# agussomacal/ROMHighContrast

Measured on AMD Instinct MI355X. Metric: snapshot_solves_per_sec, higher is better.
Workload: dtype f64

## Files before the change

romhighcontrast_amd/csrc/rom_fem_dev.h:

```cpp
#pragma once
#include "rom_fem_plan.h"
#include "rom_mma.h"

struct FemDev {
  int nrb, ncb, N, n1, n1p, nr, nc, nGp, nGa, T, nslots, kblk, npre, nrhs, nexp, ncross, xb0;
  long long dim;
  const double* pool;
  const int* alist;
  const int* aoff;
  int tile_stream;
  const int* pairs;
  int npairs;
  const double* pool_acc;
  const int* wmeta;
  int wp0[5];
  int s1_t0, s1_nterm, s1_ndr;
  const int* s1_items;
  const int* s1_citems;
  const GenTerm* terms;
  const double* Bt;
  const double* P;
  const double* vec;
  const RhsTerm* rhs;
  const PreEdge* pre;
// ... 33 lines not shown
  const int* colti;
  const BlockSide* sides;
  int n_lr;
  const int* lr_blocks;
  const int* gen_blocks;
  const int* vmap;
  const int* scat;
  int nscat;
  double* L;
  double* invL;
  double* y;
  int* status;
};


FemDev make_dev(const rom_fem* f);

constexpr int S1_COEF_BYTES = 4 * COEF_MAX * 8, S1_WAVE_BYTES = (40 * 64 + 64 * 4 + 64 + 64 + 3 * 64 * 4) * 8;
constexpr int S1_ITEM_PASSES = 4;
constexpr int S1_DENSE_BYTES = 64 * 64 * 8;
constexpr int S1_LDS_BYTES = S1_COEF_BYTES + 4 * S1_WAVE_BYTES + S1_DENSE_BYTES;

__global__ void k_repack_table(const double* __restrict__ G, int ld, int nseg, int n1, int orient, double* __restrict__ Gs);
__global__ void k_build_A0(double* A0, const double* Qp, const double* rho, int n1, int n1p, int N);
__global__ void k_rhs(FemDev f, const double* __restrict__ a);
__global__ void k_coef(FemDev f, const double* __restrict__ a);
__global__ void k_expand(FemDev f, const double* __restrict__ a, int Mc, double* __restrict__ U, long long row0);
__global__ void k_back_pre(FemDev f, const double* __restrict__ a, int Mc);
template <int NS>
__global__ void k_diag_update(FemDev f, const double* __restrict__ a, int slot, int Mc);
__global__ void k_diag_factor(FemDev f, int slot, int j);
__global__ void k_solve1(FemDev f, const double* __restrict__ a, int Mc);
template <int NS>
__global__ void k_factor_panel(FemDev f, const double* __restrict__ a, int j, int Mc);
__global__ void k_backsolve(FemDev f);
__global__ void k_edge_transform(FemDev f, int Mc);
__global__ void k_extend(FemDev f, const double* __restrict__ a, int Mc, double* __restrict__ U, long long row0, const int* __restrict__ blocks, int pw_log2);
struct X128Args {
  int blocks[X128_BLOCKS];
  BlockSide sides[X128_BLOCKS];
};

template <bool FLAT>
__global__ void k_extend128(FemDev f, X128Args xa, const double* __restrict__ a, int Mc, double* __restrict__ U, long long row0, int with_expand, int sys_fast);
__device__ inline void load4_any(const double* __restrict__ p, double v[4]) {
  if (p) {
// ... 64 lines not shown
```

romhighcontrast_amd/csrc/rom_fem_kernels.hip:

```cpp
#include "rom_fem_dev.h"

__global__ void k_build_A0(double* A0, const double* Qp, const double* rho, int n1, int n1p, int N) {
  size_t idx = blockIdx.x * size_t(blockDim.x) + threadIdx.x;
  size_t total = size_t(n1) * n1 * n1p;
  if (idx >= total) return;
  int m = int(idx % n1p);
  size_t ij = idx / n1p;
  int j = int(ij % n1) + 1, i = int(ij / n1) + 1;
  A0[idx] = (m < n1) ? Qp[size_t(j - 1) * n1p + m] * rho[size_t(m) * (N + 1) + i] : 0.0;
}

__global__ void k_repack_table(const double* __restrict__ G, int ld, int nseg, int n1, int orient, double* __restrict__ Gs) {
  const long long idx = blockIdx.x * (long long)blockDim.x + threadIdx.x;
  const long long hrows = (long long)n1 * n1;
  if (idx >= (long long)nseg * hrows * 8) return;
  const int kk = int(idx & 7);
  const long long rp = (idx >> 3) % hrows, seg = (idx >> 3) / hrows;
  const long long row = orient ? (rp % n1) * n1 + rp / n1 : rp;
  const int k = int(seg) * 8 + kk;
  Gs[idx] = k < ld ? G[row * ld + k] : 0.0;
}


__device__ inline double readlane_f64(double v, int lane) {
  int lo = __builtin_amdgcn_readlane(__double2loint(v), lane);
  int hi = __builtin_amdgcn_readlane(__double2hiint(v), lane);
  return __hiloint2double(hi, lo);
}

__device__ inline double term_coef(const GenTerm& g, const double* __restrict__ am) {
  switch (g.kind) {
    case 0: return -am[g.b[0]];
    case 1: return am[g.b[0]] + am[g.b[1]];
    case 2: return -(am[g.b[0]] + am[g.b[1]]) / 2;
    case 3: return ((am[g.b[0]] + am[g.b[1]]) + am[g.b[2]]) + am[g.b[3]];
    case 4: return -(am[g.b[0]] * am[g.b[1]] / (am[g.b[2]] + am[g.b[3]]));
    case 5: return -(am[g.b[0]] / 2);
    default: return -((am[g.b[2]] + am[g.b[3]]) / 4);
  }
}

struct STile {
  double v[16];
// ... 1416 lines not shown
    const int cidx = acc_col(wp, jb);
    const int wi = i0 + (cidx >> pw_log2) - 1, wj = j0 + (cidx & (pw - 1)) - 1;
    w_own[jb] = (wi < n1 && wj < n1) ? f.W[wi * n1 + wj] : 0.0;
  }
#pragma unroll
  for (int i = 0; i < 2; ++i)
#pragma unroll
    for (int g = 0; g < 4; ++g) {
      const int m = blockIdx.y * 64 + acc_row(wp, i, g);
      const double sc = scs[acc_row(wp, i, g)];
      const double x0 = acc.c[i][0][g] + sc * w_own[0], x1 = acc.c[i][1][g] + sc * w_own[1];
      const double got = lane_swap1(odd ? x0 : x1);
      if (m >= Mc) continue;
      double* dst = U + (row0 + m) * f.dim + gidx;
      const double lo = odd ? got : x0, hi = odd ? x1 : got;
      if (v1) *reinterpret_cast<double2_u*>(dst) = double2_u{lo, hi};
      else if (v0) dst[0] = lo;
    }
}



constexpr int X128_SLOT = 4 * 128 * 64;

template <bool FLAT>
__global__ __launch_bounds__(512, 2) void k_extend128(FemDev f, X128Args xa, const double* __restrict__ a, int Mc,
                                                      double* __restrict__ U, long long row0, int with_expand,
                                                      int sys_fast) {
  __shared__ __align__(16) char lds_bytes[2 * X128_SLOT];
  __shared__ double scs[128];
  double* const lds = reinterpret_cast<double*>(lds_bytes);
  const int n1 = f.n1, N = f.N;
  const int nct = (n1 + 127) / 128;
  const int nvert = n1 * n1;
  const int ntile = FLAT ? (nvert + 127) / 128 : n1 * nct;
  int bx, by, ngy;
  if (sys_fast > 0) {
    bx = int(blockIdx.x) / sys_fast; by = int(blockIdx.x) % sys_fast; ngy = sys_fast;
  } else if (sys_fast < 0) {
    ngy = -sys_fast;
    const int unit = int(blockIdx.x) / (8 * ngy), r = int(blockIdx.x) % (8 * ngy);
    bx = unit * 8 + (r & 7); by = r >> 3;
  } else {
    bx = int(blockIdx.x); by = int(blockIdx.y); ngy = int(gridDim.y);
  }
  if (bx >= ntile + with_expand) return;
// ... 16 lines not shown
  const BlockSide sd = xa.sides[bz];
  const int iv = bx / nct + 1;
  const int jv0 = 128 * (bx % nct) + 1;
  const int vt0 = 128 * bx;
  const int lane = threadIdx.x & 63, w = __builtin_amdgcn_readfirstlane(threadIdx.x >> 6), wr = w >> 2, wc = w & 3;
  constexpr int NJ = 2;
  const int fr = lane & 15, kq = lane >> 4;
  double my_sc = 0.0;
  if (threadIdx.x < 128) {
    const int m = by * 128 + threadIdx.x;
    if (m < Mc) my_sc = f.y[size_t(m) * f.nGp + f.sblk0 + b];
  }
  double w_own[NJ];
#pragma unroll
  for (int j = 0; j < NJ; ++j) {
    if (FLAT) {
      const int v = vt0 + wc * (16 * NJ) + j * 16 + fr;
      w_own[j] = v < nvert ? f.W[v] : 0.0;
    } else {
      const int jj = jv0 + wc * (16 * NJ) + j * 16 + fr;
      w_own[j] = jj <= n1 ? f.W[(iv - 1) * n1 + (jj - 1)] : 0.0;
    }
  }
  const int cnt0 = sd.s[0].mode == 2 ? min(2 * sd.s[0].nch, (sd.s[0].r + 1 + 7) / 8) : 0;
  const int cnt1 = sd.s[1].mode == 2 ? min(2 * sd.s[1].nch, (sd.s[1].r + 1 + 7) / 8) : 0;
  const int cnt2 = sd.s[2].mode == 2 ? min(2 * sd.s[2].nch, (sd.s[2].r + 1 + 7) / 8) : 0;
  const int cnt3 = sd.s[3].mode == 2 ? min(2 * sd.s[3].nch, (sd.s[3].r + 1 + 7) / 8) : 0;
  const int nseg = cnt0 + cnt1 + cnt2 + cnt3;
  const int tot = (nseg + 1) / 2;
  const unsigned fx = unsigned((kq >> 1) ^ (fr >> 2));
  const unsigned fa0 = unsigned(fr * 64) + (fx << 4) + unsigned(kq & 1) * 8u;
  const unsigned fa1 = unsigned(fr * 64) + ((fx ^ 2u) << 4) + unsigned(kq & 1) * 8u;
#define X_FRAGS(SLOT_, KKI_, AF_, BF_)                                                                             \
  do {                                                                                                             \
    const char* pf_ = lds_bytes + (SLOT_) * X128_SLOT + (((KKI_)&1) ? fa1 : fa0);                                  \
    const char* pa_ = pf_ + ((KKI_) >> 1) * 8192 + wr * 4096;                                                      \
    const char* pb_ = pf_ + 16384 + ((KKI_) >> 1) * 8192 + wc * (1024 * NJ);                                       \
    _Pragma("unroll") for (int i_ = 0; i_ < 4; ++i_) AF_[i_] = *reinterpret_cast<const double*>(pa_ + i_ * 1024);  \
    _Pragma("unroll") for (int i_ = 0; i_ < NJ; ++i_) BF_[i_] = *reinterpret_cast<const double*>(pb_ + i_ * 1024); \
  } while (0)
  const unsigned lds0 = unsigned(size_t((__attribute__((address_space(3))) char*)lds_bytes));
  const unsigned du16 = unsigned(((lane & 3) ^ ((lane >> 4) & 3)) * 16);
  const unsigned ybytes_row = unsigned(f.nGp) * 8u;
  const int m0 = by * 128;
  unsigned voA[2];
  int vi[2], vj[2];
#pragma unroll
  for (int g = 0; g < 2; ++g) {
    const int rl = 32 * (w & 3) + 16 * g + (lane >> 2);
    voA[g] = unsigned(max(0, min(rl, Mc - 1 - m0))) * ybytes_row + du16;
// ... 7 lines not shown
    }
  }
  const char* const ybase = reinterpret_cast<const char*>(f.y) + size_t(min(m0, Mc - 1)) * ybytes_row;
  const char* const gsbase = reinterpret_cast<const char*>(f.Gs);
  const size_t seg_stride = size_t(n1) * n1 * 64;
  const char* const zbase = reinterpret_cast<const char*>(f.W + size_t(n1) * n1);
  const unsigned voZ = unsigned(lane) * 16u;
  int c_side = -1, c_left = 0, c_segs = nseg;
  const char* pA = zbase;
  const char* pB = zbase;
  unsigned voB[2] = {0, 0};
#define X_NEXT_SIDE()                                                                                              \
  do {                                                                                                             \
    do {                                                                                                           \
      ++c_side;                                                                                                    \
      c_left = c_side == 0 ? cnt0 : c_side == 1 ? cnt1 : c_side == 2 ? cnt2 : cnt3;                                \
    } while (c_left == 0 && c_side < 3);                                                                           \
    const int off_ = c_side == 0 ? sd.s[0].off : c_side == 1 ? sd.s[1].off : c_side == 2 ? sd.s[2].off : sd.s[3].off; \
    const int gseg_ = c_side == 0 ? sd.s[0].gseg : c_side == 1 ? sd.s[1].gseg : c_side == 2 ? sd.s[2].gseg : sd.s[3].gseg; \
     \
         \
    const int ci_ = c_side == 1 ? -n1 : n1, cj_ = c_side == 3 ? -1 : 1;                                             \
    const int k0_ = c_side == 1 ? n1 * n1 - 1 : c_side == 3 ? -n1 + n1 : -n1 - 1;                                   \
    pA = ybase + size_t(off_) * 8;                                                                                 \
    pB = gsbase + size_t(gseg_) * 8;                                                                               \
    voB[0] = unsigned(ci_ * vi[0] + cj_ * vj[0] + k0_) * 64u + du16;                                               \
    voB[1] = unsigned(ci_ * vi[1] + cj_ * vj[1] + k0_) * 64u + du16;                                               \
  } while (0)
#define X_DMA(LDS_, BASE_, VOFF_)                                                                                  \
  asm volatile("s_mov_b32 m0, %0\n\tglobal_load_lds_dwordx4 %1, %2" ::"s"(__builtin_amdgcn_readfirstlane(LDS_)),   \
               "v"(VOFF_), "s"(x128_uniform(BASE_))                                                                \
               : "memory", "m0")
#define X_ISSUE_HALF(SLOT_, H_, MINE_)                                                                             \
  do {                                                                                                             \
    const unsigned sb_ = lds0 + unsigned(SLOT_) * X128_SLOT + (H_) * 8192 + unsigned(w & 3) * 2048;                \
    if (c_segs > 0) {                                                                                              \
      if (MINE_) {                                                                                                 \
        X_DMA(sb_, pA, voA[0]);                                                                                    \
        X_DMA(sb_ + 1024, pA, voA[1]);                                                                             \
        X_DMA(sb_ + 16384, pB, voB[0]);                                                                            \
        X_DMA(sb_ + 16384 + 1024, pB, voB[1]);                                                                     \
      }                                                                                                            \
      pA += 64;                                                                                                    \
      pB += seg_stride;                                               \
      --c_segs;                                                                                                    \
      if (--c_left == 0 && c_segs > 0) X_NEXT_SIDE();                                                              \
    } else if (MINE_) {                                                 \
      X_DMA(sb_, zbase, voZ);                                                                                      \
// ... 148 lines not shown
```

romhighcontrast_amd/csrc/rom_fem_plan.h:

```cpp
#pragma once
#include <string>
#include <vector>

#include "romhc_internal.h"

constexpr int COEF_MAX = 64;
#ifndef PAIR_RING_
#define PAIR_RING_ 8
#endif
constexpr int PAIR_RING = PAIR_RING_;
constexpr int DENSE_GROUPS_MAX = 8;
constexpr int EXT_ZERO_PAGE = 256;
constexpr int X128_BLOCKS = 16;

__host__ __device__ inline int h0_row(int s, int i, int j, int N, int n1) {
  int ii, jj;
  switch (s) {
    case 0: ii = i; jj = j; break;
    case 1: ii = N - i; jj = j; break;
    case 2: ii = j; jj = i; break;
    default: ii = N - j; jj = i; break;
  }
  return (ii - 1) * n1 + (jj - 1);
}

struct FemSwitches {
  bool no_preelim, no_compress, no_lowrank_ext, no_ext_lr, verbose;
  long double compress_tol;
};

struct FemPlan {
  int nrb, ncb, N, n1, n1p, nr, nc, nG, nGp, nGa, nred, ncross, xb0, T, nslots, n_all_edges, npre_all;
  int64_t dim;
  int spos0, nsc, npairs = 0, wp0[5] = {}, ncoef, ncf, nctask, ndg, ndi, n_edges, lr_nch;
  bool fused1 = false;
  std::vector<double> pool, pool_acc, dmat, Ptab, Bt, Qp, rho, Wz, g_red, vecs, cm;
  std::vector<GenTerm> terms;
  std::vector<TileDesc> desc;
  std::vector<int> alist, aoff, pairs, wmeta, s1_items, s1_citems, dweight, ditem_group, ditem_k, kmax, item_group, item_k, item_cf;
  std::vector<int> ctask, xred, scb, kptr, kpair, colptr, colrow, colti, vmap, scat, lr_blocks, gen_blocks, epos;
  std::vector<DenseGroup> dgroups;
  std::vector<RhsTerm> rhs_terms;
  std::vector<PreEdge> pre_edges;
  std::vector<ExpEdge> exps;
  std::vector<CoefGroup> groups;
  std::vector<BlockSide> sides;
  struct GemmG { std::vector<double> Bh; long long off; int rp; };
  struct Repack { long long goff, gsoff; int ld, nseg, orient; };
  std::vector<GemmG> gemm_G;
  std::vector<Repack> repacks;
  long long gtotal = 0, gstotal = 0;
  std::vector<int> ranks, slot_of, diag_slot;
  double ext_flops = 0, flops_solve = 0, bytes_solve = 0;
};

int rom_fem_plan(int nrb, int ncb, int N, const FemSwitches& sw, FemPlan* out, std::string* error);
```

romhighcontrast_amd/csrc/rom_fem_plan.hip:

```cpp
#include "rom_fem_plan.h"

#include <algorithm>
#include <array>
#include <atomic>
#include <chrono>
#include <cmath>
#include <cstring>
#include <map>
#include <set>
#include <thread>
#include <tuple>

#include "rom_hostla.h"

namespace {

using hostla::ld;
using hostla::Mat;

struct Edge {
  int hv, p, q;
  int b0, b1;
};

struct Small {
  int rpos, cpos;
  Mat tab;
  int kind;
  std::array<int, 4> b;
};

struct Comp {
  int r = 0;
  Mat W;
  Mat Kt;
  Mat P;
  std::vector<ld> gt;
  std::vector<ld> p0;
  Mat KiW;
  std::vector<ld> wK;
};

template <class F>
void parallel_for(size_t n, F fn) {
  const unsigned nthr = std::max(1u, std::min<unsigned>(std::thread::hardware_concurrency(), unsigned(n)));
  std::atomic<size_t> next{0};
  auto work = [&]() {
    for (size_t i = next++; i < n; i = next++) fn(i);
  };
  std::vector<std::thread> pool;
  for (unsigned t = 1; t < nthr; ++t) pool.emplace_back(work);
  work();
  for (auto& th : pool) th.join();
}

struct UnitBlock {
  int N, n1;
  Mat Q, rho;
  std::vector<ld> lam, kappa;
  Mat Wl;
  Mat Kmat, Kinv;
  std::vector<ld> gE[2];
  std::vector<double> rho_d, Wd;
// ... 122 lines not shown
  }
  Mat Wb(n1, r);
  for (int i = 0; i < n1; ++i)
    for (int k = 0; k < r; ++k) Wb(i, k) = Wfull(i, k);
  cp.r = r;
  cp.W = Wb;
  Mat KiW = hostla::mul(ub.Kinv, Wb);
  Mat G = hostla::mul_tn(Wb, KiW);
  for (int i = 0; i < G.r; ++i)
    for (int j = 0; j < i; ++j) G(i, j) = G(j, i) = (G(i, j) + G(j, i)) / 2;
  if (!hostla::spd_inverse(G, cp.Kt)) return false;
  cp.P = hostla::mul(KiW, cp.Kt);
  std::vector<ld> v = hostla::matvec(ub.Kinv, ub.gE[hv]);
  std::vector<ld> wv = hostla::matvec(hostla::transpose(Wb), v);
  cp.gt = hostla::matvec(cp.Kt, wv);
  std::vector<ld> pw = hostla::matvec(cp.P, wv);
  cp.p0.resize(n1);
  for (int i = 0; i < n1; ++i) cp.p0[i] = v[i] - pw[i];
  cp.KiW = KiW;
  cp.wK = v;
  return true;
}

struct TermAcc {
  std::array<int, 5> key;
  std::vector<double> tab;
  int r_lo, r_hi, c_lo, c_hi;
};

void put_table(std::vector<double>& pool, size_t idx, int n1p, const Mat& A, bool transposed) {
  double* dst = pool.data() + idx * size_t(n1p) * n1p;
  for (int i = 0; i < A.r; ++i)
    for (int j = 0; j < A.c; ++j) {
      if (transposed) dst[size_t(j) * n1p + i] = double(A(i, j));
      else dst[size_t(i) * n1p + j] = double(A(i, j));
    }
}

int pad_bk(int r) { return (r + 1 + BK - 1) / BK * BK; }
int segs8(int r) { return (r + 1 + 7) / 8; }

int push_vec(std::vector<double>& vecs, const std::vector<ld>& v, int padded) {
  const int off = int(vecs.size());
  for (ld x : v) vecs.push_back(double(x));
  for (int i = int(v.size()); i < padded; ++i) vecs.push_back(0.0);
  return off;
// ... 118 lines not shown
    for (int e = 0; e < E; ++e) {
      if (done[e] || is_pre[e]) continue;
      if (best < 0 || g[e].size() < bd) { best = e; bd = g[e].size(); }
    }
    done[best] = 1;
    el.ord_of[best] = int(el.order.size());
    el.order.push_back(best);
    std::vector<int> nb(g[best].begin(), g[best].end());
    for (int x : nb) {
      g[x].erase(best);
      for (int y : nb)
        if (x != y) g[x].insert(y);
    }
  }
  return el;
}

struct Compression {
  std::vector<std::vector<int>> sigs;
  std::vector<int> comp_of;
  std::vector<Comp> comps;
  std::vector<int> kmax, rp;
  std::vector<char> use_lr;
  double kavg = 0;
};

void edge_types(const Topology& t, Compression& c) {
  std::map<std::vector<int>, int> sig_id;
  c.comp_of.assign(t.E, -1);
  for (int e = 0; e < t.E; ++e) {
    const Edge& ed = t.edges[e];
    std::vector<int> sig{ed.hv};
    for (int blk : {ed.b0, ed.b1}) {
      const int sf = t.side_of(blk, e);
      for (int s2 = 0; s2 < 4; ++s2)
        if (s2 != sf && t.bside[blk][s2] >= 0) sig.push_back(sf * 4 + s2);
    }
    bool x0 = false, x1 = false;
    for (auto& x : t.xc)
      if (x.edge == e) (x.node == 0 ? x0 : x1) = true;
    sig.push_back(100 + (x0 ? 1 : 0) + (x1 ? 2 : 0));
    auto it = sig_id.find(sig);
    if (it == sig_id.end()) {
      it = sig_id.emplace(sig, int(c.sigs.size())).first;
      c.sigs.push_back(sig);
    }
    c.comp_of[e] = it->second;
  }
}

bool compress_edges(UnitBlock& ub, const Topology& t, const Elimination& el, const FemSwitches& sw, Compression& c) {
  const int n1 = t.n1;
  const bool compress = !sw.no_compress;
  const ld ctol = sw.compress_tol, ckeep = std::min<ld>(ctol, 1e-17L);
  const size_t ntype = c.sigs.size();
  c.comps.resize(ntype);
  std::vector<int> ids, ids_tk;
  for (auto& sig : c.sigs)
    for (size_t k = 1; k + 1 < sig.size(); ++k) ids.push_back(sig[k]);
  for (int e : el.pre_list)
    for (int u : t.adj[e]) {
      ids_tk.push_back(t.table_id(u, e));
      ids.push_back(t.table_id(e, u));
    }
  ub.prepare(ids, false);
  ub.prepare(ids_tk, true);
  std::vector<char> ok(ntype, 1);
  std::vector<Mat> Wfull(ntype);
  std::vector<std::vector<ld>> pivots(ntype);
  if (compress)
    parallel_for(ntype, [&](size_t k) {
      const std::vector<int>& sig = c.sigs[k];
      const int flags = sig.back() - 100;
      compress_basis(ub, std::vector<int>(sig.begin() + 1, sig.end() - 1), flags & 1, flags & 2, ckeep, Wfull[k], pivots[k]);
    });
  std::vector<int> r_drop(ntype, n1), r_use(ntype, n1);
  if (compress) {
    std::vector<int> r_fill(ntype, n1);
    for (size_t k = 0; k < ntype; ++k) {
      int r = 0;
      while (r < int(pivots[k].size()) && pivots[k][r] > ctol * pivots[k][0]) ++r;
      r_drop[k] = r;
      r_fill[k] = std::min<int>(int(pivots[k].size()), segs8(r) * 8 - 1);
    }
    auto tiles = [&](const std::vector<int>& rr) {
      long long nred = t.ncross;
      for (int e : el.order) nred += std::min(rr[c.comp_of[e]], n1);
      return (nred + TB - 1) / TB;
    };
    r_use = tiles(r_fill) <= tiles(r_drop) ? r_fill : r_drop;
  }
  parallel_for(ntype, [&](size_t k) { ok[k] = compress_finish(ub, Wfull[k], r_use[k], c.sigs[k][0], compress, c.comps[k]); });
  return std::find(ok.begin(), ok.end(), 0) == ok.end();
}

void extension_ranks(const UnitBlock& ub, int n1p, bool no_lowrank_ext, Compression& c) {
  const int N = ub.N, n1 = ub.n1;
  c.kmax.assign(N + 1, n1p);
  for (int dd = 1; dd <= N; ++dd) {
    int last = -1;
    for (int m = 0; m < n1; ++m)
      if (ub.rho_d[size_t(m) * (N + 1) + std::min(dd, N)] >= 1e-18) last = m;
    c.kmax[dd] = std::min(n1p, std::max(BK, (last + 1 + BK - 1) / BK * BK));
    if (dd <= n1) c.kavg += c.kmax[dd] / double(std::max(n1, 1));
  }
  c.kmax[0] = n1p;
  c.rp.assign(c.comps.size(), 0);
  c.use_lr.assign(c.comps.size(), 0);
  for (size_t k = 0; k < c.comps.size(); ++k) {
    c.rp[k] = pad_bk(c.comps[k].r);
    c.use_lr[k] = c.comps[k].r < n1 && c.rp[k] <= 1.25 * c.kavg && n1 > 0 && !no_lowrank_ext;
  }
}

struct Layout {
// ... 574 lines not shown
  for (int it = 0; it < p.ncoef; ++it) {
    const CoefGroup& cg = groups[p.item_group[it]];
    const int k = p.item_k[it];
    const int code = cg.kind == 1 && k < cg.r ? 0 : k == cg.r ? 1 : k < cg.r ? 2 : 3;
    int* r = &p.s1_citems[size_t(it) * 4];
    r[0] = (cg.cpos + k) | code << 28; r[1] = cg.zpos + k; r[2] = cg.b0; r[3] = cg.b1;
  }
}

void unit_block_tables(UnitBlock& ub, const BtTables& bt, FemPlan& p) {
  const int n1 = p.n1, n1p = p.n1p;
  p.Bt.assign(std::max<size_t>(size_t(bt.n) * n1p * n1p, 1), 0.0);
  for (auto& kv : bt.of_id) put_table(p.Bt, kv.second, n1p, ub.TK(kv.first), true);
  for (auto& kv : bt.extra) put_table(p.Bt, kv.first, n1p, kv.second, false);
  p.Qp.assign(size_t(n1p) * n1p, 0.0);
  for (int j = 0; j < n1; ++j)
    for (int m = 0; m < n1; ++m) p.Qp[size_t(j) * n1p + m] = double(ub.Q(j, m));
  p.rho = ub.rho_d;
  p.Wz = ub.Wd;
  p.Wz.resize(ub.Wd.size() + EXT_ZERO_PAGE, 0.0);
}

using GOffsets = std::map<std::pair<int, int>, long long>;
GOffsets g_tables(const UnitBlock& ub, const Topology& t, const Elimination& el, const Compression& c, const Layout& L, FemPlan& p) {
  const int n1 = t.n1, n1p = p.n1p;
  GOffsets goff;
  for (int e = 0; e < t.E; ++e)
    if (L.cpos[e] >= 0 && !goff.count({c.comp_of[e], int(el.is_pre[e])})) {
      goff[{c.comp_of[e], int(el.is_pre[e])}] = p.gtotal;
      p.gtotal += (long long)n1 * n1 * c.rp[c.comp_of[e]];
    }
  for (auto& kv : goff) p.gemm_G.push_back({{}, kv.second, c.rp[kv.first.first]});
  std::vector<std::pair<int, int>> gkeys;
  for (auto& kv : goff) gkeys.push_back(kv.first);
  parallel_for(gkeys.size(), [&](size_t gi) {
    const Comp& cp = c.comps[gkeys[gi].first];
    const Mat& Pm = gkeys[gi].second == 0 ? cp.P : cp.KiW;
    const std::vector<ld>& pv = gkeys[gi].second == 0 ? cp.p0 : cp.wK;
    Mat Bm = hostla::mul_tn(Pm, ub.Q);
    std::vector<double>& Bh = p.gemm_G[gi].Bh;
    Bh.assign(size_t(p.gemm_G[gi].rp) * n1p, 0.0);
    for (int k = 0; k < cp.r; ++k)
      for (int m = 0; m < n1; ++m) Bh[size_t(k) * n1p + m] = double(Bm(k, m));
    for (int m = 0; m < n1; ++m) {
      ld sacc = 0;
      for (int k = 0; k < n1; ++k) sacc += pv[k] * ub.Q(k, m);
      Bh[size_t(cp.r) * n1p + m] = double(sacc);
    }
  });
  return goff;
}

void extension_sides(const Topology& t, const Elimination& el, const Compression& c, const Layout& L, const GOffsets& goff, FemPlan& p) {
  const int n1 = t.n1, N = t.N;
  const long long hrows = (long long)n1 * n1;
  p.sides.resize(t.nrb * t.ncb);
  std::map<std::tuple<int, int, int>, long long> gsoff;
  std::vector<char> need_tr(t.E, 0);
  double fl = 0;
  const int npj = (n1 + 15) / 16, npi = (n1 + 3) / 4;
  for (int b = 0; b < t.nrb * t.ncb; ++b)
    for (int sdx = 0; sdx < 4; ++sdx) {
      ExtSide& es = p.sides[b].s[sdx];
      memset(&es, 0, sizeof(es));
      const int e = t.bside[b][sdx];
      if (e < 0) continue;
      const int k = c.comp_of[e], r = c.comps[k].r;
      if (L.cpos[e] >= 0) {
        es = ExtSide{2, L.cpos[e], c.rp[k] / BK, r, int(goff.at({k, int(el.is_pre[e])})), 0, t.edges[e].b0, t.edges[e].b1};
        const auto key = std::make_tuple(k, int(el.is_pre[e]), sdx >= 2 ? 1 : 0);
        if (!gsoff.count(key)) {
          gsoff[key] = p.gstotal;
          p.gstotal += (long long)segs8(r) * hrows * 8;
        }
        es.gseg = int(gsoff[key]);
        fl += 2.0 * double(n1) * n1 * (r + 1);
      } else {
        es.mode = 1;
        es.off = L.npos[e];
        need_tr[e] = 1;
        for (int pi = 0; pi < npi; ++pi)
          for (int pj = 0; pj < npj; ++pj) {
            int i0 = 4 * pi + 1, j0 = 16 * pj + 1, i1 = std::min(i0 + 3, n1), j1 = std::min(j0 + 15, n1);
            int dist[4] = {i0, N - i1, j0, N - j1};
            fl += 2.0 * 64 * c.kmax[dist[sdx]];
          }
      }
    }
  for (auto& kv : gsoff) {
    const int k = std::get<0>(kv.first);
    p.repacks.push_back({goff.at({k, std::get<1>(kv.first)}), kv.second, c.rp[k], segs8(c.comps[k].r), std::get<2>(kv.first)});
  }
  for (int e = 0; e < t.E; ++e)
    if (need_tr[e]) p.epos.push_back(L.npos[e]);
  p.n_edges = int(p.epos.size());
  if (p.epos.empty()) p.epos.push_back(0);
  p.ext_flops = fl + 2.0 * p.n_edges * double(p.n1p) * p.n1p;
}

// ... 21 lines not shown
    fprintf(stderr, "romhc:   tile assembly as a stream: %zu KB per system and sweep in pieces of 8 rows x 16 columns\n", real);
  }
  {
    double strips = 0, tiles_diag = 0, tiles_sub = 0, nterm = 0;
    for (const TileDesc& d : p.desc) {
      (d.ti == d.tj ? tiles_diag : tiles_sub) += 1;
      for (int t = d.t0; t < d.t1; ++t) {
        const GenTerm& g = p.terms[t];
        nterm += 1;
        for (int r = g.r_lo; r < g.r_hi; ++r)
          for (int c0 = 0; c0 < 64; c0 += 16)
            if (c0 < g.c_hi && c0 + 16 > g.c_lo) strips += 1;
      }
    }
    fprintf(stderr, "romhc:   tile assembly: %.0f diagonal + %.0f sub-diagonal tiles, %.0f terms, %.1f KB of table strips per system and sweep\n",
            tiles_diag, tiles_sub, nterm, strips * 128 / 1024);
  }
  fprintf(stderr, "romhc: %dx%d blocks N=%d: %d edges (%d closed-form, %d of them compressed), reduced size %d -> %d tiles, "
                  "%d slots, %zu terms, kavg %.1f\n", p.nrb, p.ncb, p.N, p.n_all_edges, p.npre_all, p.npre_all - int(p.pre_edges.size()),
          p.nred, p.T, p.nslots, p.terms.size(), c.kavg);
  for (size_t k = 0; k < c.comps.size(); ++k)
    fprintf(stderr, "romhc:   edge type %zu: rank %d (padded %d), %d edges, extension %s\n", k, c.comps[k].r, c.rp[k],
            int(std::count(c.comp_of.begin(), c.comp_of.end(), int(k))), c.use_lr[k] ? "from the reduced unknowns" : "sine modes");
  fprintf(stderr, "romhc:   blocks extended by the 128-tile kernel: %d, general kernel: %d\n", int(p.lr_blocks.size()), int(p.gen_blocks.size()));
  size_t nzb = 0, rect = 0, rows16 = 0;
  for (const GenTerm& g : p.terms) {
    const double* tb = p.pool.data() + size_t(g.tab) * 4096;
    rect += size_t(g.r_hi - g.r_lo) * size_t(g.c_hi - g.c_lo);
    for (int ib = 0; ib < 4; ++ib)
      for (int jb = 0; jb < 4; ++jb) {
        bool nz = false;
        for (int i = 0; i < 16 && !nz; ++i)
          for (int j = 0; j < 16; ++j)
            if (tb[(16 * ib + i) * 64 + 16 * jb + j] != 0.0) { nz = true; break; }
        nzb += nz;
      }
    for (int r = 0; r < 64; ++r)
      for (int sg = 0; sg < 4; ++sg) {
        bool nz = false;
        for (int j = 0; j < 16; ++j) nz = nz || tb[r * 64 + 16 * sg + j] != 0.0;
        rows16 += nz;
      }
  }
  const size_t nt = p.terms.size();
  fprintf(stderr, "romhc:   term tables: %zu tables, %zu non-zero 16x16 blocks of %zu (%.2f), bounding rectangles cover %.2f, non-zero 1x16 strips %.2f\n",
          nt, nzb, nt * 16, double(nzb) / (nt * 16), double(rect) / (nt * 4096.0), double(rows16) / (nt * 256.0));
// ... 14 lines not shown
}

int rom_fem_plan(int nrb, int ncb, int N, const FemSwitches& sw, FemPlan* out, std::string* error) {
  FemPlan& p = *out;
  p = FemPlan();
  auto fail = [&](const char* why) { *error = why; return ROM_ERR_INVALID; };
  PhaseTimer phase{sw.verbose};
  phase.next("topology");
  const Topology t = make_topology(nrb, ncb, N);
  const int n1 = N - 1, n1p = (n1 + TB - 1) / TB * TB;
  p.nrb = nrb; p.ncb = ncb; p.N = N; p.n1 = n1; p.n1p = n1p;
  p.nr = nrb * N - 1;
  p.nc = ncb * N - 1;
  p.dim = int64_t(p.nr) * p.nc;
  p.nG = t.E * n1 + t.ncross;
  p.ncross = t.ncross;
  p.n_all_edges = t.E;
  phase.next("elimination order");
  const Elimination el = choose_elimination(t, sw.no_preelim);
  p.npre_all = int(el.pre_list.size());
  phase.next("unit-block tables in long double, compression of the edges");
  UnitBlock ub(N, t.E > 0);
  Compression c;
  edge_types(t, c);
  if (!compress_edges(ub, t, el, sw, c)) return fail("internal: compressed edge block not positive definite");
  extension_ranks(ub, n1p, sw.no_lowrank_ext, c);
  p.kmax = c.kmax;
  phase.next("layout of the interface vector");
  const Layout L = make_layout(t, el, c, n1p);
  p.nred = L.nred; p.T = L.T; p.nGa = L.nGa; p.xb0 = L.xb0; p.nGp = L.nGp; p.spos0 = L.spos0; p.nsc = L.nsc;
  p.xred = L.xred;
  for (int e : el.order) p.ranks.push_back(L.rk[e]);
  std::vector<Small> smalls;
  BtTables bt;
  double pre_flops;
  {
    phase.next("W^T T products");
    const WtCache wt = wt_products(ub, t, el, c, L);
    phase.next("blocks of the reduced matrix");
    smalls = reduced_blocks(t, el, c, L, wt);
    phase.next("closed-form edges");
    pre_flops = closed_form_records(closed_form_products(ub, t, el, c, L, wt), t, el, c, L, p, smalls, bt);
    if (pre_flops < 0) return fail("internal: more than 8 neighbours of an eliminated edge");
  }
  phase.next("tile mask + symbolic fill");
  std::vector<std::pair<int, int>> slots;
  const double chol_flops = symbolic_cholesky(smalls, L.T, p, slots);
// ... 26 lines not shown
```

romhighcontrast_amd/csrc/rom_fem_setup.hip:

```cpp
#include <algorithm>
#include <cstdlib>
#include <memory>

#include "rom_fem_dev.h"

#ifdef ROMHC_AB
static const char* ab_env(const char* name) { return getenv(name); }
#else
static const char* ab_env(const char*) { return nullptr; }
#endif

FemDev make_dev(const rom_fem* f) {
  FemDev d;
  d.nrb = f->nrb; d.ncb = f->ncb; d.N = f->N; d.n1 = f->n1; d.n1p = f->n1p; d.nr = f->nr; d.nc = f->nc;
  d.nGp = f->nGp; d.nGa = f->nGa; d.T = f->T; d.nslots = f->nslots; d.kblk = f->nrb * f->ncb; d.npre = f->npre;
  d.nrhs = f->nrhs; d.nexp = f->nexp; d.ncross = f->ncross; d.xb0 = f->xb0; d.dim = f->dim;
  d.pool = f->d_pool; d.alist = f->d_alist; d.aoff = f->d_aoff; d.tile_stream = f->sw_no_tile_stream ? 0 : 1;
  d.pairs = f->d_pairs; d.npairs = f->npairs; d.pool_acc = f->d_pool_acc; d.wmeta = f->d_wmeta;
  for (int i = 0; i < 5; ++i) d.wp0[i] = f->wp0[i];
  d.s1_t0 = d.s1_nterm = d.s1_ndr = 0;
  if (f->fused1 && !f->desc.empty()) {
    d.s1_t0 = f->desc[0].t0; d.s1_nterm = f->desc[0].t1 - f->desc[0].t0; d.s1_ndr = f->desc[0].ndr;
  }
  d.s1_items = f->d_s1_items; d.s1_citems = f->d_s1_citems; d.terms = f->d_terms;
// ... 39 lines not shown
  return ROM_OK;
}

int build_extension_tables(rom_fem* f, const FemPlan& p) {
  rom_ctx* ctx = f->ctx;
  const int n1 = p.n1, n1p = p.n1p;
  const size_t hrows = size_t(n1) * n1;
  ROM_TRY(dev_alloc(f->tables, &f->d_A0, hrows * n1p));
  if (hrows > 0) {
    TempTables tmp;
    double* d_rho = nullptr;
    ROM_TRY(upload(ctx->stream, tmp.list, &d_rho, p.rho));
    k_build_A0<<<unsigned((hrows * n1p + 255) / 256), 256, 0, ctx->stream>>>(f->d_A0, f->d_Qp, d_rho, n1, n1p, p.N);
    ROM_HIP(hipGetLastError());
    ROM_HIP(hipStreamSynchronize(ctx->stream));
  }
  ROM_TRY(dev_alloc(f->tables, &f->d_G, size_t(p.gtotal)));
  for (const FemPlan::GemmG& g : p.gemm_G) {
    TempTables tmp;
    double* d_B = nullptr;
    ROM_TRY(upload(ctx->stream, tmp.list, &d_B, g.Bh));
    ROM_TRY(rom_launch_gemm_nt(ctx, int64_t(hrows), g.rp, n1p, 1.0, f->d_A0, n1p, d_B, n1p, 0.0, f->d_G + g.off, g.rp,
                               "setup_gemm_G"));
    ROM_HIP(hipStreamSynchronize(ctx->stream));
  }
  ROM_TRY(dev_alloc(f->tables, &f->d_Gs, size_t(p.gstotal)));
  f->gs_bytes = size_t(p.gstotal) * sizeof(double);
  for (const FemPlan::Repack& r : p.repacks) {
    const size_t total = size_t(r.nseg) * hrows * 8;
    if (total == 0) continue;
    k_repack_table<<<unsigned((total + 255) / 256), 256, 0, ctx->stream>>>(f->d_G + r.goff, r.ld, r.nseg, n1, r.orient,
                                                                            f->d_Gs + r.gsoff);
    ROM_HIP(hipGetLastError());
  }
  ROM_HIP(hipStreamSynchronize(ctx->stream));
  return ROM_OK;
}

}

extern "C" int rom_fem_destroy(rom_fem* f) {
  if (!f) return ROM_OK;
  hipStreamSynchronize(f->ctx->stream);
  for (void* p : f->tables) hipFree(p);
  void* lazy[] = {f->d_L, f->d_invL, f->d_y, f->d_yhat, f->d_dots, f->d_riesz, f->d_green};
  for (void* p : lazy)
    if (p) hipFree(p);
  rom_factored_map_free(f->fmap);
  delete f;
  return ROM_OK;
}

extern "C" int rom_fem_create(rom_ctx* ctx, int nrb, int ncb, int N, rom_fem** out) {
  ROM_CHECK(ctx && out, "rom_fem_create: null argument");
  ROM_CHECK(nrb >= 1 && ncb >= 1 && N >= 2, "rom_fem_create: need nrb,ncb >= 1 and N >= 2 (got %d,%d,%d)", nrb, ncb, N);
  ROM_CHECK(nrb * ncb <= 64, "rom_fem_create: at most 64 blocks supported (got %d)", nrb * ncb);
  ROM_HIP(hipSetDevice(ctx->device));
  FemSwitches sw;
  sw.no_preelim = getenv("ROMHC_NO_PREELIM") != nullptr;
  sw.no_compress = getenv("ROMHC_NO_COMPRESS") != nullptr;
  sw.no_lowrank_ext = getenv("ROMHC_NO_LOWRANK_EXT") != nullptr;
  sw.no_ext_lr = ab_env("ROMHC_NO_EXT_LR") != nullptr;
  sw.verbose = getenv("ROMHC_VERBOSE") != nullptr;
  sw.compress_tol = 1e-14L;
  if (const char* s = getenv("ROMHC_COMPRESS_TOL")) sw.compress_tol = (long double)atof(s);
  FemPlan p;
  std::string why;
  if (rom_fem_plan(nrb, ncb, N, sw, &p, &why) != ROM_OK) {
    rom_set_error("%s", why.c_str());
    return ROM_ERR_INVALID;
  }
  std::unique_ptr<rom_fem, int (*)(rom_fem*)> guard(new rom_fem(), rom_fem_destroy);
  rom_fem* f = guard.get();
  f->ctx = ctx;
  f->nrb = nrb; f->ncb = ncb; f->N = N; f->n1 = p.n1; f->n1p = p.n1p; f->nr = p.nr; f->nc = p.nc; f->dim = p.dim;
  f->nG = p.nG; f->nGp = p.nGp; f->nGa = p.nGa; f->nred = p.nred; f->ncross = p.ncross; f->xb0 = p.xb0; f->T = p.T;
  f->nslots = p.nslots; f->npre = int(p.pre_edges.size()); f->nexp = int(p.exps.size()); f->nrhs = int(p.rhs_terms.size());
  f->spos0 = p.spos0; f->nsc = p.nsc; f->n_all_edges = p.n_all_edges; f->npairs = p.npairs; f->fused1 = p.fused1;
  for (int i = 0; i < 5; ++i) f->wp0[i] = p.wp0[i];
  f->ncoef = p.ncoef; f->ncf = p.ncf; f->nctask = p.nctask; f->ndg = p.ndg; f->ndi = p.ndi; f->n_edges = p.n_edges;
  f->n_lr_blocks = int(p.lr_blocks.size()); f->n_gen_blocks = int(p.gen_blocks.size()); f->lr_nch = p.lr_nch;
  f->nscat = int(p.scat.size()); f->ext_flops = p.ext_flops; f->flops_solve = p.flops_solve; f->bytes_solve = p.bytes_solve;
  f->desc = p.desc; f->slot_of = p.slot_of; f->kptr = p.kptr; f->kpair = p.kpair; f->colptr = p.colptr; f->colrow = p.colrow;
  f->colti = p.colti; f->diag_slot = p.diag_slot; f->sides = p.sides; f->ranks = p.ranks; f->lr_blocks_host = p.lr_blocks;
#define ROM_UPLOAD(member, vec) ROM_TRY(upload(ctx->stream, f->tables, &f->member, p.vec))
  ROM_UPLOAD(d_pool, pool);         ROM_UPLOAD(d_terms, terms);           ROM_UPLOAD(d_desc, desc);
  ROM_UPLOAD(d_alist, alist);       ROM_UPLOAD(d_aoff, aoff);             ROM_UPLOAD(d_pairs, pairs);
  ROM_UPLOAD(d_pool_acc, pool_acc); ROM_UPLOAD(d_wmeta, wmeta);           ROM_UPLOAD(d_s1_items, s1_items);
// ... 30 lines not shown
```

romhighcontrast_amd/csrc/rom_hostla.h:

```cpp
#pragma once
#include <algorithm>
#include <cmath>
#include <cstddef>
#include <thread>
#include <vector>

namespace hostla {

typedef long double ld;

struct Mat {
  int r = 0, c = 0;
  std::vector<ld> v;
  Mat() {}
  Mat(int r_, int c_) : r(r_), c(c_), v(size_t(r_) * c_, 0.0L) {}
  ld& operator()(int i, int j) { return v[size_t(i) * c + j]; }
  ld operator()(int i, int j) const { return v[size_t(i) * c + j]; }
  ld* row(int i) { return v.data() + size_t(i) * c; }
  const ld* row(int i) const { return v.data() + size_t(i) * c; }
};

inline Mat transpose(const Mat& A) {
  Mat B(A.c, A.r);
  for (int i = 0; i < A.r; ++i)
// ... 159 lines not shown
    ++rank;
  }
  Mat Wt(rank, n);
  for (int j = 0; j < rank; ++j) Wt(j, j) = 1.0L;
  for (int k = rank - 1; k >= 0; --k) {
    const std::vector<ld>& v = refl[k];
    for (int j = 0; j < rank; ++j) {
      ld* wj = Wt.row(j);
      ld s = 0;
      for (int i = k; i < n; ++i) s += v[i] * wj[i];
      s *= 2;
      for (int i = k; i < n; ++i) wj[i] -= s * v[i];
    }
  }
  return transpose(Wt);
}

inline Mat identity(int n) {
  Mat I(n, n);
  for (int i = 0; i < n; ++i) I(i, i) = 1.0L;
  return I;
}

}
```

romhighcontrast_amd/csrc/romhc_internal.h:

```cpp
#pragma once
#include <hip/hip_runtime.h>

#include <cstdarg>
#include <cstdint>
#include <cstdio>
#include <map>
#include <string>
#include <vector>

#include "romhc.h"

void rom_set_error(const char* fmt, ...);

#define ROM_HIP(call)                                                                      \
  do {                                                                                     \
    hipError_t _e = (call);                                                                \
    if (_e != hipSuccess) {                                                                \
      rom_set_error("%s failed: %s (%s:%d)", #call, hipGetErrorString(_e), __FILE__, __LINE__); \
      return ROM_ERR_HIP;                                                                  \
    }                                                                                      \
  } while (0)

#define ROM_CHECK(cond, ...)      \
  do {                            \
// ... 84 lines not shown

struct GenTerm {
  int tab;
  short r_lo, r_hi, c_lo, c_hi;
  int kind;
  int b[4];
};

struct TileDesc {
  int ti, tj;
  int t0, t1;
  int ndr;
  int diag;
};

struct ExtSide {
  int mode;
  int off;
  int nch;
  int r;
  int gtab;
  int gseg;
  int b0, b1;
};
struct DenseGroup {
  int cpos, r, b0, b1;
  int nv;
  int voff[4], vblk[4], vu0[4], vu1[4];
};

struct BlockSide {
  ExtSide s[4];
};

struct RhsTerm {
  int pos, len, voff, kind, b0, e0, e1;
};

struct PreNb {
  int fpos;
  int blk;
  int nch;
  int bt;
};
struct PreEdge {
  int pos;
// ... 139 lines not shown
```

Before: 4.197 million.

## Rotate edge bases to echelon form and skip negligible extension K segments

```diff
diff --git a/romhighcontrast_amd/csrc/rom_fem_dev.h b/romhighcontrast_amd/csrc/rom_fem_dev.h
--- a/romhighcontrast_amd/csrc/rom_fem_dev.h
+++ b/romhighcontrast_amd/csrc/rom_fem_dev.h
@@ -79,6 +79,8 @@
 constexpr int S1_LDS_BYTES = S1_COEF_BYTES + 4 * S1_WAVE_BYTES + S1_DENSE_BYTES;
 
 __global__ void k_repack_table(const double* __restrict__ G, int ld, int nseg, int n1, int orient, double* __restrict__ Gs);
+struct ExtThresholds { unsigned short thr[8]; };
+__global__ void k_mask_table(double* __restrict__ G, int ld, int n1, ExtThresholds th);
 __global__ void k_build_A0(double* A0, const double* Qp, const double* rho, int n1, int n1p, int N);
 __global__ void k_rhs(FemDev f, const double* __restrict__ a);
 __global__ void k_coef(FemDev f, const double* __restrict__ a);
diff --git a/romhighcontrast_amd/csrc/rom_fem_kernels.hip b/romhighcontrast_amd/csrc/rom_fem_kernels.hip
--- a/romhighcontrast_amd/csrc/rom_fem_kernels.hip
+++ b/romhighcontrast_amd/csrc/rom_fem_kernels.hip
@@ -19,6 +19,15 @@
   const long long row = orient ? (rp % n1) * n1 + rp / n1 : rp;
   const int k = int(seg) * 8 + kk;
   Gs[idx] = k < ld ? G[row * ld + k] : 0.0;
+}
+
+__global__ void k_mask_table(double* __restrict__ G, int ld, int n1, ExtThresholds th) {
+  const long long idx = blockIdx.x * (long long)blockDim.x + threadIdx.x;
+  if (idx >= (long long)n1 * n1 * ld) return;
+  const int k = int(idx % ld), d = int(idx / ld / n1) + 1;
+  int skip = 0;
+  for (int j = 0; j < EXT_THRESHOLDS; ++j) skip += d >= int(th.thr[j]) ? 1 : 0;
+  if (k < 8 * skip) G[idx] = 0.0;
 }
 
 
@@ -1481,6 +1490,14 @@
 
 
 constexpr int X128_SLOT = 4 * 128 * 64;
+static_assert(sizeof(FemDev) + sizeof(X128Args) + 64 <= 4096, "k_extend128's arguments must fit the kernel argument segment");
+
+__device__ inline int x128_skip(const ExtSide& s, int d) {
+  int n = 0;
+#pragma unroll
+  for (int j = 0; j < EXT_THRESHOLDS; ++j) n += d >= int(s.thr[j]) ? 1 : 0;
+  return n;
+}
 
 template <bool FLAT>
 __global__ __launch_bounds__(512, 2) void k_extend128(FemDev f, X128Args xa, const double* __restrict__ a, int Mc,
@@ -1543,10 +1560,30 @@
       w_own[j] = jj <= n1 ? f.W[(iv - 1) * n1 + (jj - 1)] : 0.0;
     }
   }
-  const int cnt0 = sd.s[0].mode == 2 ? min(2 * sd.s[0].nch, (sd.s[0].r + 1 + 7) / 8) : 0;
-  const int cnt1 = sd.s[1].mode == 2 ? min(2 * sd.s[1].nch, (sd.s[1].r + 1 + 7) / 8) : 0;
-  const int cnt2 = sd.s[2].mode == 2 ? min(2 * sd.s[2].nch, (sd.s[2].r + 1 + 7) / 8) : 0;
-  const int cnt3 = sd.s[3].mode == 2 ? min(2 * sd.s[3].nch, (sd.s[3].r + 1 + 7) / 8) : 0;
+  int dist0, dist1, dist2, dist3;
+  if (FLAT) {
+    const int vend = min(vt0 + 127, nvert - 1), i_lo = vt0 / n1, i_hi = vend / n1;
+    const bool one_row = i_lo == i_hi;
+    dist0 = i_lo + 1;
+    dist1 = N - (i_hi + 1);
+    dist2 = one_row ? vt0 - i_lo * n1 + 1 : 1;
+    dist3 = one_row ? N - (vend - i_hi * n1 + 1) : 1;
+  } else {
+    dist0 = iv;
+    dist1 = N - iv;
+    dist2 = jv0;
+    dist3 = N - min(jv0 + 127, n1);
+  }
+#define X_SEGS(S_) min(2 * sd.s[S_].nch, (sd.s[S_].r + 1 + 7) / 8)
+  const int sk0 = sd.s[0].mode == 2 ? min(x128_skip(sd.s[0], dist0), X_SEGS(0) - 1) : 0;
+  const int sk1 = sd.s[1].mode == 2 ? min(x128_skip(sd.s[1], dist1), X_SEGS(1) - 1) : 0;
+  const int sk2 = sd.s[2].mode == 2 ? min(x128_skip(sd.s[2], dist2), X_SEGS(2) - 1) : 0;
+  const int sk3 = sd.s[3].mode == 2 ? min(x128_skip(sd.s[3], dist3), X_SEGS(3) - 1) : 0;
+  const int cnt0 = sd.s[0].mode == 2 ? X_SEGS(0) - sk0 : 0;
+  const int cnt1 = sd.s[1].mode == 2 ? X_SEGS(1) - sk1 : 0;
+  const int cnt2 = sd.s[2].mode == 2 ? X_SEGS(2) - sk2 : 0;
+  const int cnt3 = sd.s[3].mode == 2 ? X_SEGS(3) - sk3 : 0;
+#undef X_SEGS
   const int nseg = cnt0 + cnt1 + cnt2 + cnt3;
   const int tot = (nseg + 1) / 2;
   const unsigned fx = unsigned((kq >> 1) ^ (fr >> 2));
@@ -1600,8 +1637,9 @@
          \
     const int ci_ = c_side == 1 ? -n1 : n1, cj_ = c_side == 3 ? -1 : 1;                                             \
     const int k0_ = c_side == 1 ? n1 * n1 - 1 : c_side == 3 ? -n1 + n1 : -n1 - 1;                                   \
-    pA = ybase + size_t(off_) * 8;                                                                                 \
-    pB = gsbase + size_t(gseg_) * 8;                                                                               \
+    const int sk_ = c_side == 0 ? sk0 : c_side == 1 ? sk1 : c_side == 2 ? sk2 : sk3;         \
+    pA = ybase + size_t(off_) * 8 + size_t(sk_) * 64;                                                              \
+    pB = gsbase + size_t(gseg_) * 8 + size_t(sk_) * seg_stride;                                                    \
     voB[0] = unsigned(ci_ * vi[0] + cj_ * vj[0] + k0_) * 64u + du16;                                               \
     voB[1] = unsigned(ci_ * vi[1] + cj_ * vj[1] + k0_) * 64u + du16;                                               \
   } while (0)
diff --git a/romhighcontrast_amd/csrc/rom_fem_plan.h b/romhighcontrast_amd/csrc/rom_fem_plan.h
--- a/romhighcontrast_amd/csrc/rom_fem_plan.h
+++ b/romhighcontrast_amd/csrc/rom_fem_plan.h
@@ -11,6 +11,8 @@
 constexpr int PAIR_RING = PAIR_RING_;
 constexpr int DENSE_GROUPS_MAX = 8;
 constexpr int EXT_ZERO_PAGE = 256;
+constexpr int EXT_THRESHOLDS = 7;
+constexpr long double EXT_TRUNC_CUT = 1e-18L;
 constexpr int X128_BLOCKS = 16;
 
 __host__ __device__ inline int h0_row(int s, int i, int j, int N, int n1) {
@@ -27,6 +29,7 @@
 struct FemSwitches {
   bool no_preelim, no_compress, no_lowrank_ext, no_ext_lr, verbose;
   long double compress_tol;
+  bool no_ext_trunc;
 };
 
 struct FemPlan {
@@ -45,7 +48,14 @@
   std::vector<ExpEdge> exps;
   std::vector<CoefGroup> groups;
   std::vector<BlockSide> sides;
-  struct GemmG { std::vector<double> Bh; long long off; int rp; };
+  struct GemmG {
+    std::vector<double> Bh; long long off; int rp;
+    int r = 0;
+    std::vector<int> entry, seg0;
+    std::vector<long double> W;
+    unsigned short thr[8] = {0xffff, 0xffff, 0xffff, 0xffff, 0xffff, 0xffff, 0xffff, 0xffff};
+    double cut = 0;
+  };
   struct Repack { long long goff, gsoff; int ld, nseg, orient; };
   std::vector<GemmG> gemm_G;
   std::vector<Repack> repacks;
diff --git a/romhighcontrast_amd/csrc/rom_fem_plan.hip b/romhighcontrast_amd/csrc/rom_fem_plan.hip
--- a/romhighcontrast_amd/csrc/rom_fem_plan.hip
+++ b/romhighcontrast_amd/csrc/rom_fem_plan.hip
@@ -39,6 +39,7 @@
   std::vector<ld> p0;
   Mat KiW;
   std::vector<ld> wK;
+  std::vector<int> entry;
 };
 
 template <class F>
@@ -207,6 +208,19 @@
   return true;
 }
 
+bool rotate_to_echelon(const UnitBlock& ub, int hv, int variant, Comp& cp) {
+  const int n1 = ub.n1, r = cp.r;
+  std::vector<int> entry;
+  const Mat E = hostla::echelon_rotation(hostla::mul_tn(variant == 0 ? cp.P : cp.KiW, ub.Q), &entry);
+  const Mat WE = hostla::mul(cp.W, E);
+  Mat Wr(n1, r);
+  for (int i = 0; i < n1; ++i)
+    for (int k = 0; k < r; ++k) Wr(i, k) = WE(i, r - 1 - k);
+  if (!compress_finish(ub, Wr, r, hv, true, cp)) return false;
+  cp.entry.assign(entry.rbegin(), entry.rend());
+  return true;
+}
+
 struct TermAcc {
   std::array<int, 5> key;
   std::vector<double> tab;
@@ -371,10 +385,11 @@
   std::vector<Comp> comps;
   std::vector<int> kmax, rp;
   std::vector<char> use_lr;
+  std::vector<char> variant;
   double kavg = 0;
 };
 
-void edge_types(const Topology& t, Compression& c) {
+void edge_types(const Topology& t, const Elimination& el, bool by_variant, Compression& c) {
   std::map<std::vector<int>, int> sig_id;
   c.comp_of.assign(t.E, -1);
   for (int e = 0; e < t.E; ++e) {
@@ -388,11 +403,13 @@
     bool x0 = false, x1 = false;
     for (auto& x : t.xc)
       if (x.edge == e) (x.node == 0 ? x0 : x1) = true;
-    sig.push_back(100 + (x0 ? 1 : 0) + (x1 ? 2 : 0));
+    const int variant = by_variant && el.is_pre[e] ? 1 : 0;
+    sig.push_back(100 + (x0 ? 1 : 0) + (x1 ? 2 : 0) + 4 * variant);
     auto it = sig_id.find(sig);
     if (it == sig_id.end()) {
       it = sig_id.emplace(sig, int(c.sigs.size())).first;
       c.sigs.push_back(sig);
+      c.variant.push_back(char(variant));
     }
     c.comp_of[e] = it->second;
   }
@@ -439,7 +456,10 @@
     };
     r_use = tiles(r_fill) <= tiles(r_drop) ? r_fill : r_drop;
   }
-  parallel_for(ntype, [&](size_t k) { ok[k] = compress_finish(ub, Wfull[k], r_use[k], c.sigs[k][0], compress, c.comps[k]); });
+  parallel_for(ntype, [&](size_t k) {
+    ok[k] = compress_finish(ub, Wfull[k], r_use[k], c.sigs[k][0], compress, c.comps[k]);
+    if (ok[k] && compress && !sw.no_ext_trunc && c.comps[k].r < n1) ok[k] = rotate_to_echelon(ub, c.sigs[k][0], c.variant[k], c.comps[k]);
+  });
   return std::find(ok.begin(), ok.end(), 0) == ok.end();
 }
 
@@ -1060,6 +1080,32 @@
 }
 
 using GOffsets = std::map<std::pair<int, int>, long long>;
+
+void ext_truncation(const UnitBlock& ub, const Comp& cp, int n1p, FemPlan::GemmG& g) {
+  const int n1 = ub.n1, N = ub.N, r = cp.r, nseg = segs8(r);
+  g.entry = cp.entry;
+  g.W = cp.W.v;
+  for (int k = 0; k < r; ++k)
+    for (int m = 0; m < std::min(cp.entry[k], n1); ++m) g.Bh[size_t(k) * n1p + m] = 0.0;
+  auto bound = [&](int k, int d) {
+    ld b = 0;
+    for (int m = 0; m < n1; ++m) b += ub.rho(m, d) * fabsl(ld(g.Bh[size_t(k) * n1p + m]));
+    return b;
+  };
+  ld top = 0;
+  for (int k = 0; k < r; ++k) top = std::max(top, bound(k, 1));
+  const ld cut = EXT_TRUNC_CUT * top;
+  g.cut = double(cut);
+  for (int d = 1; d <= n1; ++d) {
+    int first = 0;
+    while (first < r && bound(first, d) < cut) ++first;
+    g.seg0[d] = std::min({first / 8, nseg - 1, EXT_THRESHOLDS});
+  }
+  g.seg0[N] = g.seg0[n1];
+  for (int j = 0; j < EXT_THRESHOLDS; ++j)
+    for (int d = n1; d >= 1; --d)
+      if (g.seg0[d] > j) g.thr[j] = (unsigned short)d;
+}
 GOffsets g_tables(const UnitBlock& ub, const Topology& t, const Elimination& el, const Compression& c, const Layout& L, FemPlan& p) {
   const int n1 = t.n1, n1p = p.n1p;
   GOffsets goff;
@@ -1085,6 +1131,9 @@
       for (int k = 0; k < n1; ++k) sacc += pv[k] * ub.Q(k, m);
       Bh[size_t(cp.r) * n1p + m] = double(sacc);
     }
+    p.gemm_G[gi].r = cp.r;
+    p.gemm_G[gi].seg0.assign(t.N + 1, 0);
+    if (!cp.entry.empty()) ext_truncation(ub, cp, n1p, p.gemm_G[gi]);
   });
   return goff;
 }
@@ -1105,14 +1154,22 @@
       if (e < 0) continue;
       const int k = c.comp_of[e], r = c.comps[k].r;
       if (L.cpos[e] >= 0) {
-        es = ExtSide{2, L.cpos[e], c.rp[k] / BK, r, int(goff.at({k, int(el.is_pre[e])})), 0, t.edges[e].b0, t.edges[e].b1};
+        es = ExtSide{2, L.cpos[e], c.rp[k] / BK, r, int(goff.at({k, int(el.is_pre[e])})), 0, t.edges[e].b0, t.edges[e].b1, {}};
         const auto key = std::make_tuple(k, int(el.is_pre[e]), sdx >= 2 ? 1 : 0);
         if (!gsoff.count(key)) {
           gsoff[key] = p.gstotal;
           p.gstotal += (long long)segs8(r) * hrows * 8;
         }
         es.gseg = int(gsoff[key]);
-        fl += 2.0 * double(n1) * n1 * (r + 1);
+        const FemPlan::GemmG* gg = nullptr;
+        for (const FemPlan::GemmG& cand : p.gemm_G)
+          if (cand.off == es.gtab) gg = &cand;
+        memcpy(es.thr, gg->thr, sizeof(es.thr));
+        if (gg->entry.empty()) {
+          fl += 2.0 * double(n1) * n1 * (r + 1);
+        } else {
+          for (int d = 1; d <= n1; ++d) fl += 2.0 * double(n1) * (r + 1 - 8 * gg->seg0[d]);
+        }
       } else {
         es.mode = 1;
         es.off = L.npos[e];
@@ -1180,6 +1237,14 @@
   for (size_t k = 0; k < c.comps.size(); ++k)
     fprintf(stderr, "romhc:   edge type %zu: rank %d (padded %d), %d edges, extension %s\n", k, c.comps[k].r, c.rp[k],
             int(std::count(c.comp_of.begin(), c.comp_of.end(), int(k))), c.use_lr[k] ? "from the reduced unknowns" : "sine modes");
+  for (size_t i = 0; i < p.gemm_G.size(); ++i) {
+    const FemPlan::GemmG& g = p.gemm_G[i];
+    const int full = segs8(g.r);
+    long long need = 0;
+    for (int d = 1; d <= p.n1; ++d) need += full - g.seg0[d];
+    fprintf(stderr, "romhc:   extension table %zu: rank %d, %s basis, K segments needed %lld of %lld (%.2f)\n", i, g.r,
+            g.entry.empty() ? "pivoted" : "echelon", need, (long long)full * p.n1, p.n1 > 0 ? double(need) / (double(full) * p.n1) : 1.0);
+  }
   fprintf(stderr, "romhc:   blocks extended by the 128-tile kernel: %d, general kernel: %d\n", int(p.lr_blocks.size()), int(p.gen_blocks.size()));
   size_t nzb = 0, rect = 0, rows16 = 0;
   for (const GenTerm& g : p.terms) {
@@ -1240,7 +1305,7 @@
   phase.next("unit-block tables in long double, compression of the edges");
   UnitBlock ub(N, t.E > 0);
   Compression c;
-  edge_types(t, c);
+  edge_types(t, el, !sw.no_ext_trunc && !sw.no_compress, c);
   if (!compress_edges(ub, t, el, sw, c)) return fail("internal: compressed edge block not positive definite");
   extension_ranks(ub, n1p, sw.no_lowrank_ext, c);
   p.kmax = c.kmax;
diff --git a/romhighcontrast_amd/csrc/rom_fem_setup.hip b/romhighcontrast_amd/csrc/rom_fem_setup.hip
--- a/romhighcontrast_amd/csrc/rom_fem_setup.hip
+++ b/romhighcontrast_amd/csrc/rom_fem_setup.hip
@@ -1,5 +1,6 @@
 #include <algorithm>
 #include <cstdlib>
+#include <cstring>
 #include <memory>
 
 #include "rom_fem_dev.h"
@@ -85,6 +86,12 @@
     ROM_TRY(upload(ctx->stream, tmp.list, &d_B, g.Bh));
     ROM_TRY(rom_launch_gemm_nt(ctx, int64_t(hrows), g.rp, n1p, 1.0, f->d_A0, n1p, d_B, n1p, 0.0, f->d_G + g.off, g.rp,
                                "setup_gemm_G"));
+    if (!g.entry.empty() && hrows > 0) {
+      ExtThresholds th;
+      memcpy(th.thr, g.thr, sizeof(th.thr));
+      k_mask_table<<<unsigned((hrows * g.rp + 255) / 256), 256, 0, ctx->stream>>>(f->d_G + g.off, g.rp, n1, th);
+      ROM_HIP(hipGetLastError());
+    }
     ROM_HIP(hipStreamSynchronize(ctx->stream));
   }
   ROM_TRY(dev_alloc(f->tables, &f->d_Gs, size_t(p.gstotal)));
@@ -127,6 +134,7 @@
   sw.verbose = getenv("ROMHC_VERBOSE") != nullptr;
   sw.compress_tol = 1e-14L;
   if (const char* s = getenv("ROMHC_COMPRESS_TOL")) sw.compress_tol = (long double)atof(s);
+  sw.no_ext_trunc = getenv("ROMHC_NO_EXT_TRUNC") != nullptr;
   FemPlan p;
   std::string why;
   if (rom_fem_plan(nrb, ncb, N, sw, &p, &why) != ROM_OK) {
diff --git a/romhighcontrast_amd/csrc/rom_hostla.h b/romhighcontrast_amd/csrc/rom_hostla.h
--- a/romhighcontrast_amd/csrc/rom_hostla.h
+++ b/romhighcontrast_amd/csrc/rom_hostla.h
@@ -1,5 +1,6 @@
 #pragma once
 #include <algorithm>
+#include <cfloat>
 #include <cmath>
 #include <cstddef>
 #include <thread>
@@ -205,4 +206,49 @@
   return I;
 }
 
-}
+inline Mat echelon_rotation(const Mat& C, std::vector<int>* entry) {
+  const int r = C.r, n = C.c;
+  Mat A = C;
+  ld scale = 0;
+  for (ld x : A.v) scale += x * x;
+  scale = sqrtl(scale);
+  std::vector<std::vector<ld>> refl;
+  entry->assign(r, n);
+  int k = 0;
+  for (int m = 0; m < n && k < r; ++m) {
+    ld s = 0;
+    for (int i = k; i < r; ++i) s += A(i, m) * A(i, m);
+    s = sqrtl(s);
+    if (!(s > 1e3L * LDBL_EPSILON * scale)) continue;
+    std::vector<ld> v(r, 0.0L);
+    const ld alpha = A(k, m) > 0 ? -s : s;
+    ld vn = 0;
+    for (int i = k; i < r; ++i) {
+      v[i] = A(i, m) - (i == k ? alpha : 0.0L);
+      vn += v[i] * v[i];
+    }
+    vn = sqrtl(vn);
+    for (int i = k; i < r && vn > 0.0L; ++i) v[i] /= vn;
+    for (int j = m; j < n; ++j) {
+      ld d = 0;
+      for (int i = k; i < r; ++i) d += v[i] * A(i, j);
+      d *= 2;
+      for (int i = k; i < r; ++i) A(i, j) -= d * v[i];
+    }
+    refl.push_back(v);
+    (*entry)[k++] = m;
+  }
+  Mat E = identity(r);
+  for (int q = int(refl.size()) - 1; q >= 0; --q) {
+    const std::vector<ld>& v = refl[q];
+    for (int j = 0; j < r; ++j) {
+      ld d = 0;
+      for (int i = q; i < r; ++i) d += v[i] * E(i, j);
+      d *= 2;
+      for (int i = q; i < r; ++i) E(i, j) -= d * v[i];
+    }
+  }
+  return E;
+}
+
+}
diff --git a/romhighcontrast_amd/csrc/romhc_internal.h b/romhighcontrast_amd/csrc/romhc_internal.h
--- a/romhighcontrast_amd/csrc/romhc_internal.h
+++ b/romhighcontrast_amd/csrc/romhc_internal.h
@@ -130,6 +130,7 @@
   int gtab;
   int gseg;
   int b0, b1;
+  unsigned short thr[8];
 };
 struct DenseGroup {
   int cpos, r, b0, b1;
```

New measurement: 4.255 million (median of 6 runs). 1.01x the previous value.
